# Youngju-Na/UFORecon

Measured on AMD Instinct MI355X. Metric: rays/s (per-ray volume-rendering path, 64+64 hierarchical samples, DTU-shaped 3-view 512x640), higher is better.
Workload: dtype f32; 1 GPU; configs[1]: full 512x640 frame = 327680 rays, 3 source views, 64+64 samples, rays sharded by row tiles over 1 GPU(s), depth/RGB tiles all-gathered; rays_per_frame=327680, chunk_rays=4096, side_streams=3

## Files before the change

uforecon_amd/csrc/view_transformer.hip:

```cpp
#include <cstdlib>
#include "bwd_tape.h"
#include "ufr_internal.h"
#include "weight_stream_f16.h"

namespace ufr {

template <class T>
__device__ __forceinline__ T* at32(T* base, unsigned elem) {
  typedef typename std::conditional<std::is_const<T>::value, const char, char>::type B;
  return reinterpret_cast<T*>(reinterpret_cast<B*>(base) + (elem * (unsigned)sizeof(T)));
}

template <int C, int N>
__device__ __forceinline__ void zero_tiles(f32x4 (&t)[C][N]) {
#pragma unroll
  for (int c = 0; c < C; ++c)
#pragma unroll
    for (int i = 0; i < N; ++i) t[c][i] = splat4(0.f);
}

template <int C, int VW, int VB, class WS>
__device__ __forceinline__ void layer_norm80(f32x4 (&t)[C][5], const WS& ws, int g, float eps, float asc, f32x4 (*XH)[5] = nullptr, float* RS = nullptr) {
#pragma unroll
  for (int c = 0; c < C; ++c) {
    float s = 0.f;
#pragma unroll
    for (int i = 0; i < 5; ++i) s += (t[c][i][0] + t[c][i][1]) + (t[c][i][2] + t[c][i][3]);
    const float mean = sum_groups(s) * (1.f / 80.f);
    float q = 0.f;
#pragma unroll
    for (int i = 0; i < 5; ++i)
#pragma unroll
      for (int r = 0; r < 4; ++r) {
        float d = t[c][i][r] - mean;
        q = fmaf(d, d, q);
      }
    const float rstd = fast_rsqrt(sum_groups(q) * (1.f / 80.f) + eps);
    if (RS) RS[c] = rstd * asc;
#pragma unroll
    for (int i = 0; i < 5; ++i) {
      const f32x4 gw = vec_frag<VW>(ws, i, g), gb = vec_frag<VB>(ws, i, g);
#pragma unroll
      for (int r = 0; r < 4; ++r) {
        const float xh = (t[c][i][r] - mean) * rstd;
        if (XH) XH[c][i][r] = xh;
        t[c][i][r] = xh * gw[r] + gb[r];
      }
    }
  }
}

constexpr int kVtBlock = 256;
constexpr int kVtC = 2;
constexpr int kVtMinW = 2;
constexpr int kVtOversub = 4;
constexpr int kVtWaves = kVtBlock / 64;
#ifdef UFR_PHASE_TIMING
__device__ unsigned long long g_vt_phase[32];
__device__ unsigned long long g_vt_wave[4096 * 2];
#define UFR_PHASE(i)                                                                   \
  {                                                                                    \
    const unsigned long long t_now = __builtin_readcyclecounter();                     \
    ph_acc[i] += t_now - t_prev;                                                       \
    t_prev = t_now;                                                                    \
  }
#else
#define UFR_PHASE(i)
#endif

template <int L, int C, bool LOWP, bool TAPE = false>
__global__ void __launch_bounds__(kVtBlock, kVtMinW) view_transformer_kernel(const float* __restrict__ packed,
                                                                             const float* __restrict__ x_tokens,
                                                                             const float* __restrict__ x_point,
                                                                             const float* __restrict__ rgbm,
                                                                             const float* __restrict__ dirs, int P,
                                                                             float* __restrict__ token0,
                                                                             float* __restrict__ radiance,
                                                                             float* __restrict__ view_out,
                                                                             int* __restrict__ status,
                                                                             float* __restrict__ tape = nullptr) {
  constexpr int NV = L - 1;
  constexpr int PPT = 16 / L;
  constexpr bool STRADDLE = (L == 6 && C == 2 && !TAPE);
  static_assert(!TAPE || kBlockCols % C == 0, "tape blocks");
  constexpr int PPW = STRADDLE ? 5 : PPT * C;
  constexpr bool kScoresHook = L == 4 && C == 2 && !TAPE;
  static_assert(!kScoresHook || ksteps(M_VT_V) * mat_desc(M_VT_V).n_out >= 6 * C, "the v GEMM has too few hook slots for the scores");
  extern __shared__ __attribute__((aligned(16))) char smem[];
  auto ws = wstream_f16_begin<kVtWaves, LOWP>(packed, smem);
  wstream_f16_prime<B_VT, kVtWaves>(ws);
  const int lane = threadIdx.x & 63, g = lane >> 4, j = lane & 15;
  constexpr bool kLocalScalars = (L == 6 && C == 2 && !TAPE);
  const auto sc = scalar_file<kLocalScalars, view_scalars_offset()>(ws);
  int ptw[C], tvv[C];
  bool okc[C];
#pragma unroll
  for (int c = 0; c < C; ++c) {
    if constexpr (STRADDLE) {
      ptw[c] = j < 12 ? 3 * c + j / 6 : 2;
      tvv[c] = j < 12 ? j % 6 : (c == 0 ? j - 12 : j - 8);
      okc[c] = c == 0 || j < 14;
    } else {
      ptw[c] = c * PPT + j / L;
      tvv[c] = j % L;
      okc[c] = j < PPT * L;
    }
  }
  int src[8];
#pragma unroll
  for (int s = 0; s < 8; ++s) src[s] = okc[0] ? (lane - tvv[0] + (tvv[0] + s) % L) : lane;
  int srcx[C][5];
  if constexpr (STRADDLE) {
    constexpr int kStep[6][5] = {{4, 5, 1, 2, 3}, {4, 5, 0, 2, 3}, {4, 5, 0, 1, 3}, {4, 5, 0, 1, 2}, {5, 0, 1, 2, 3}, {4, 0, 1, 2, 3}};
#pragma unroll
    for (int c = 0; c < C; ++c)
#pragma unroll
      for (int st = 0; st < 5; ++st) {
        int u = 0;
#pragma unroll
        for (int t = 0; t < 6; ++t) u = tvv[c] == t ? kStep[t][st] : u;
        const int base = j < 12 ? (j / 6) * 6 : 12;
        const int off = j < 12 ? u : (u & 3);
        srcx[c][st] = 4 * (okc[c] ? 16 * g + base + off : lane);
      }
  }
  auto exch = [&](auto ci, auto sti, float xc, float xo) __attribute__((always_inline)) -> float {
    constexpr int c = decltype(ci)::value, st = decltype(sti)::value;
    float m = xc;
    if constexpr (c == 0 && st == 0) m = j == 12 ? xo : xc;
    if constexpr (c == 0 && st == 1) m = j == 13 ? xo : xc;
    if constexpr (c == 1 && st >= 1) m = j >= 12 ? xo : xc;
    return __builtin_bit_cast(float, __builtin_amdgcn_ds_bpermute(srcx[c][st], __builtin_bit_cast(int, m)));
  };

  const int wave_global = (blockIdx.x * blockDim.x + threadIdx.x) >> 6;
  const int n_waves = (gridDim.x * blockDim.x) >> 6;
  const int n_groups = TAPE ? ((P + PPT * kBlockCols - 1) / (PPT * kBlockCols)) * (kBlockCols / C) : (P + PPW - 1) / PPW;
  const int n_iter = (n_groups + n_waves - 1) / n_waves;

#ifdef UFR_PHASE_TIMING
  unsigned long long ph_acc[12] = {};
  unsigned long long t_prev = __builtin_readcyclecounter();
  const unsigned long long t_start = t_prev;
  const unsigned long long rt_start = __builtin_amdgcn_s_memrealtime();
#endif
  for (int it = 0; it < n_iter; ++it) {
    const int grp = it * n_waves + wave_global;
    const bool wrap = it + 1 < n_iter;
    typedef ViewTapeLayout<LOWP> TapeL;
    const int col0 = __builtin_amdgcn_readfirstlane(grp < n_groups ? grp : 0) * C;
    char* const tape_blk = reinterpret_cast<char*>(tape) + (size_t)(col0 / kBlockCols) * (TapeL::block_units * 512);
    auto tape_st = [&](int tile, int c, f32x4 v) __attribute__((always_inline)) {
      if (grp < n_groups) tile_store<TapeL>(tape_blk, tile, col0 % kBlockCols + c, lane, v);
    };
    f32x4 x[C][5];
    int pidx[C];
    bool valid[C];
    auto load_x = [&](int c, f32x4 (&dst)[5]) __attribute__((always_inline)) {
      const int pp = valid[c] ? pidx[c] : 0;
      const int tv = tvv[c];
      const unsigned vrow = ((unsigned)pp * NV + (tv > 0 ? tv - 1 : 0)) * (x_point ? kViewCols : UFR_TOKEN_DIM);
      const unsigned prow_e = x_point ? (unsigned)pp * kPointCols : vrow + 32;
      const float* pbase = x_point ? x_point : x_tokens;
      const float* row = at32(x_tokens, vrow + 4 * g);
      const float* prow = at32(pbase, prow_e + 4 * g);
      const float* last = g < 2 ? prow + 32 : row + (x_point ? 32 : 72) - 8;
#pragma unroll
      for (int t = 0; t < 5; ++t) {
        f32x4 tok = vec_frag<V_VIEW_TOKEN>(ws, t, g);
        f32x4 val = ld4(t < 2 ? row + 16 * t : t < 4 ? prow + 16 * (t - 2) : last);
        dst[t] = tv == 0 ? tok : val;
        if (!valid[c]) dst[t] = splat4(0.f);
      }
    };
#pragma unroll
    for (int c = 0; c < C; ++c) {
      pidx[c] = grp * PPW + ptw[c];
      valid[c] = okc[c] && grp < n_groups && pidx[c] < P;
      load_x(c, x[c]);
    }
    track_external(x, ws);
    if constexpr (TAPE) {
#pragma unroll
      for (int c = 0; c < C; ++c)
#pragma unroll
        for (int t = 0; t < 5; ++t) tape_st(TV_X + t, c, x[c][t]);
    }
    UFR_PHASE(0)
    f32x4 q[C][5], k[C][5];
    zero_tiles(q); zero_tiles(k);
    {
      BWords<C> cur;
      const float xs_x = sc[VS_XS_X];
      split_units<0, 0, 4 * C>(x, cur, xs_x);
      static_for<3>([&](auto si) __attribute__((always_inline)) {
        constexpr int s = decltype(si)::value;
        BStep b[C];
        bwords_to_bstep(cur, b);
        if constexpr (s < 2) {
          BWords<C> nxt;
          gemm_f16_panel<M_VT_Q, s, C, kVtWaves, false>(ws, b, q, wrap, [&](auto ti) __attribute__((always_inline)) {
            constexpr int to = decltype(ti)::value;
            split_units<s + 1, to * 4 * C / 5, (to + 1) * 4 * C / 5>(x, nxt, xs_x);
          });
          gemm_f16_panel<M_VT_K, s, C, kVtWaves>(ws, b, k, wrap);
          cur = nxt;
        } else {
          gemm_f16_panel<M_VT_Q, s, C, kVtWaves>(ws, b, q, wrap);
          gemm_f16_panel<M_VT_K, s, C, kVtWaves>(ws, b, k, wrap);
        }
      });
      probe_gemm(q, ws);
      probe_gemm(k, ws);
    }
    const float q_dsc = sc[VS_Q_DSC], q_l2e = sc[VS_Q_L2E], k_dsc = sc[VS_K_DSC], k_l2e = sc[VS_K_L2E];
    if constexpr (TAPE) {
#pragma unroll
      for (int c = 0; c < C; ++c)
#pragma unroll
        for (int t = 0; t < 5; ++t) {
          tape_st(TV_Q + t, c, f32x4{elu1_acc(q[c][t][0], q_dsc, q_l2e), elu1_acc(q[c][t][1], q_dsc, q_l2e), elu1_acc(q[c][t][2], q_dsc, q_l2e), elu1_acc(q[c][t][3], q_dsc, q_l2e)});
          tape_st(TV_K + t, c, f32x4{elu1_acc(k[c][t][0], k_dsc, k_l2e), elu1_acc(k[c][t][1], k_dsc, k_l2e), elu1_acc(k[c][t][2], k_dsc, k_l2e), elu1_acc(k[c][t][3], k_dsc, k_l2e)});
        }
    }
    UFR_PHASE(1)
    float A[C][2][L], Zs[C][2];
    if constexpr (STRADDLE) {
      static_for<2>([&](auto hi) __attribute__((always_inline)) {
        constexpr int hh = decltype(hi)::value;
        float Q[C][10], K[C][10], den[C];
#pragma unroll
        for (int c = 0; c < C; ++c) {
#pragma unroll
          for (int d = 0; d < 10; ++d) {
            const int s = 10 * hh + d;
            Q[c][d] = elu1_acc(q[c][s >> 2][s & 3], q_dsc, q_l2e);
            K[c][d] = elu1_acc(k[c][s >> 2][s & 3], k_dsc, k_l2e);
          }
          float a = 0.f;
#pragma unroll
          for (int d = 0; d < 10; ++d) a = fmaf(Q[c][d], K[c][d], a);
          A[c][hh][0] = a;
          den[c] = a;
        }
        static_for<5>([&](auto sti) __attribute__((always_inline)) {
          constexpr int st = decltype(sti)::value;
          float a0 = 0.f, a1 = 0.f;
#pragma unroll
          for (int d = 0; d < 10; ++d) {
            a0 = fmaf(Q[0][d], exch(std::integral_constant<int, 0>{}, sti, K[0][d], K[1][d]), a0);
            a1 = fmaf(Q[1][d], exch(std::integral_constant<int, 1>{}, sti, K[1][d], K[0][d]), a1);
          }
          A[0][hh][1 + st] = a0; den[0] += a0;
          A[1][hh][1 + st] = a1; den[1] += a1;
        });
#pragma unroll
        for (int c = 0; c < C; ++c) Zs[c][hh] = (float)L * fast_rcp(den[c] + 1e-6f);
      });
    } else if constexpr (kScoresHook) {
    } else {
#pragma unroll
    for (int c = 0; c < C; ++c) {
#pragma unroll
      for (int hh = 0; hh < 2; ++hh) {
        float Q[10], K[10];
#pragma unroll
        for (int d = 0; d < 10; ++d) {
          const int s = 10 * hh + d;
          Q[d] = elu1_acc(q[c][s >> 2][s & 3], q_dsc, q_l2e);
          K[d] = elu1_acc(k[c][s >> 2][s & 3], k_dsc, k_l2e);
        }
        float den = 0.f;
#define UFR_ATT_STEP(S)                                                  \
        if (S < L) {                                                     \
          float a = 0.f;                                                 \
          if constexpr (L == 4 && S >= 1 && S <= 3) {                    \
            a = dot10_rot4<(S >= 1 && S <= 3) ? S : 1>(Q, K);           \
          } else {                                                       \
            _Pragma("unroll") for (int d = 0; d < 10; ++d) a = fmaf(Q[d], rot<L, S>(K[d], src), a); \
          }                                                              \
          den += a;                                                      \
          A[c][hh][S < L ? S : 0] = a;                                   \
        }
        UFR_ATT_STEP(0) UFR_ATT_STEP(1) UFR_ATT_STEP(2) UFR_ATT_STEP(3)
        UFR_ATT_STEP(4) UFR_ATT_STEP(5) UFR_ATT_STEP(6) UFR_ATT_STEP(7)
#undef UFR_ATT_STEP
        Zs[c][hh] = (float)L * fast_rcp(den + 1e-6f);
      }
    }
    }
    UFR_PHASE(2)
    f32x4 v[C][5];
    zero_tiles(v);
    if constexpr (kScoresHook) {
      float Qs[10], Ks[10];
      gemm_f16<M_VT_V, C, kVtWaves>(ws, x, v, wrap, sc[VS_XS_X], [&](auto ui) __attribute__((always_inline)) {
        constexpr int slot = decltype(ui)::value, u = slot / 3, part = slot % 3;
        if constexpr (u < 2 * C) {
          constexpr int c = u / 2, hh = u % 2;
          if constexpr (part == 0) {
#pragma unroll
            for (int d = 0; d < 10; ++d) Qs[d] = elu1_acc(q[c][(10 * hh + d) >> 2][(10 * hh + d) & 3], q_dsc, q_l2e);
          } else if constexpr (part == 1) {
#pragma unroll
            for (int d = 0; d < 10; ++d) Ks[d] = elu1_acc(k[c][(10 * hh + d) >> 2][(10 * hh + d) & 3], k_dsc, k_l2e);
          } else {
            float a0 = 0.f;
#pragma unroll
            for (int d = 0; d < 10; ++d) a0 = fmaf(Qs[d], Ks[d], a0);
            const float a1 = dot10_rot4<1>(Qs, Ks), a2 = dot10_rot4<2>(Qs, Ks), a3 = dot10_rot4<3>(Qs, Ks);
            A[c][hh][0] = a0; A[c][hh][1] = a1; A[c][hh][2] = a2; A[c][hh][3] = a3;
            Zs[c][hh] = (float)L * fast_rcp((((0.f + a0) + a1) + a2) + a3 + 1e-6f);
          }
        }
      });
    } else {
      gemm_f16<M_VT_V, C, kVtWaves>(ws, x, v, wrap, sc[VS_XS_X]);
    }
    UFR_PHASE(3)
    const float v_dsc = sc[VS_V_DSC];
    const float v_mul = v_dsc / (float)L;
    if constexpr (TAPE) {
#pragma unroll
      for (int c = 0; c < C; ++c)
#pragma unroll
        for (int t = 0; t < 5; ++t) {
          f32x4 vv;
#pragma unroll
          for (int r = 0; r < 4; ++r)
            vv[r] = (L & (L - 1)) == 0 ? v[c][t][r] * v_mul : (v[c][t][r] * v_dsc) / (float)L;
          tape_st(TV_V + t, c, vv);
        }
    }
    f32x4 msg[C][5];
    if constexpr (STRADDLE) {
      static_for<2>([&](auto hi) __attribute__((always_inline)) {
        constexpr int hh = decltype(hi)::value;
        float V[C][10], acc[C][10];
#pragma unroll
        for (int c = 0; c < C; ++c)
#pragma unroll
          for (int d = 0; d < 10; ++d) {
            const int s = 10 * hh + d;
            V[c][d] = (v[c][s >> 2][s & 3] * v_dsc) / (float)L;
            acc[c][d] = A[c][hh][0] * V[c][d];
          }
        static_for<5>([&](auto sti) __attribute__((always_inline)) {
          constexpr int st = decltype(sti)::value;
#pragma unroll
          for (int d = 0; d < 10; ++d) {
            acc[0][d] = fmaf(A[0][hh][1 + st], exch(std::integral_constant<int, 0>{}, sti, V[0][d], V[1][d]), acc[0][d]);
            acc[1][d] = fmaf(A[1][hh][1 + st], exch(std::integral_constant<int, 1>{}, sti, V[1][d], V[0][d]), acc[1][d]);
          }
        });
#pragma unroll
        for (int c = 0; c < C; ++c)
#pragma unroll
          for (int d = 0; d < 10; ++d) {
            const int s = 10 * hh + d;
            msg[c][s >> 2][s & 3] = acc[c][d] * Zs[c][hh];
          }
      });
    } else {
#pragma unroll
    for (int c = 0; c < C; ++c) {
#pragma unroll
      for (int hh = 0; hh < 2; ++hh) {
        float V[10], acc[10];
#pragma unroll
        for (int d = 0; d < 10; ++d) {
          const int s = 10 * hh + d;
          V[d] = (L & (L - 1)) == 0 ? v[c][s >> 2][s & 3] * v_mul : (v[c][s >> 2][s & 3] * v_dsc) / (float)L;
          acc[d] = 0.f;
        }
#define UFR_ATT_STEP(S)                                                  \
        if (S < L) {                                                     \
          if constexpr (L == 4 && S >= 1 && S <= 3) {                    \
            axpy10_rot4<(S >= 1 && S <= 3) ? S : 1>(acc, A[c][hh][S < L ? S : 0], V); \
          } else {                                                       \
            _Pragma("unroll") for (int d = 0; d < 10; ++d) acc[d] = fmaf(A[c][hh][S < L ? S : 0], rot<L, S>(V[d], src), acc[d]); \
          }                                                              \
        }
        UFR_ATT_STEP(0) UFR_ATT_STEP(1) UFR_ATT_STEP(2) UFR_ATT_STEP(3)
        UFR_ATT_STEP(4) UFR_ATT_STEP(5) UFR_ATT_STEP(6) UFR_ATT_STEP(7)
#undef UFR_ATT_STEP
#pragma unroll
        for (int d = 0; d < 10; ++d) {
          const int s = 10 * hh + d;
          msg[c][s >> 2][s & 3] = acc[d] * Zs[c][hh];
        }
      }
    }
    }

    UFR_PHASE(4)
    if constexpr (TAPE) {
#pragma unroll
      for (int c = 0; c < C; ++c)
#pragma unroll
        for (int t = 0; t < 5; ++t) tape_st(TV_MSG + t, c, msg[c][t]);
    }
    f32x4 m[C][5];
    zero_tiles(m);
    gemm_f16<M_VT_MERGE, C, kVtWaves>(ws, msg, m, wrap, sc[VS_M_XS]);
    UFR_PHASE(5)
    float rstd1[C] = {}, rstd2[C] = {};
    if constexpr (TAPE) {
      f32x4 xh[C][5];
      layer_norm80<C, V_VT_N1W, V_VT_N1B>(m, ws, g, sc[VS_EPS1], sc[VS_M_ASC], xh, rstd1);
#pragma unroll
      for (int c = 0; c < C; ++c)
#pragma unroll
        for (int t = 0; t < 5; ++t) { tape_st(TV_XH1 + t, c, xh[c][t]); tape_st(TV_M + t, c, m[c][t]); }
    } else {
      layer_norm80<C, V_VT_N1W, V_VT_N1B>(m, ws, g, sc[VS_EPS1], 1.f);
    }

    UFR_PHASE(6)
    f32x4 cat[C][10], hid[C][10], o[C][5];
#pragma unroll
    for (int c = 0; c < C; ++c)
#pragma unroll
      for (int t = 0; t < 5; ++t) { cat[c][t] = x[c][t]; cat[c][5 + t] = m[c][t]; }
    zero_tiles(hid);
    gemm_f16<M_VT_MLP0, C, kVtWaves>(ws, cat, hid, wrap, sc[VS_XS_X]);
    UFR_PHASE(7)
#pragma unroll
    for (int c = 0; c < C; ++c)
#pragma unroll
      for (int t = 0; t < 10; ++t)
#pragma unroll
        for (int r = 0; r < 4; ++r) hid[c][t][r] = relu_acc(hid[c][t][r]);
    unsigned relu_bits[C][2] = {};
    if constexpr (TAPE) {
#pragma unroll
      for (int c = 0; c < C; ++c)
#pragma unroll
        for (int t = 0; t < 10; ++t) {
          tape_st(TV_HID + t, c, hid[c][t] * sc[VS_MLP0_DSC]);
#pragma unroll
          for (int r = 0; r < 4; ++r)
            if (hid[c][t][r] > 0.f) relu_bits[c][(4 * t + r) >> 5] |= 1u << ((4 * t + r) & 31);
        }
    }
    zero_tiles(o);
    gemm_f16<M_VT_MLP2, C, kVtWaves>(ws, hid, o, wrap, sc[VS_M_MLP2]);
    f32x4 col[C];
    float dcomp[C];
#pragma unroll
    for (int c = 0; c < C; ++c) {
      col[c] = splat4(0.f);
      dcomp[c] = 0.f;
      const int tv = tvv[c];
      if (valid[c] && tv > 0) {
        col[c] = ld4(at32(rgbm, ((unsigned)pidx[c] * NV + (tv - 1)) * 4u));
        dcomp[c] = *at32(dirs, ((unsigned)pidx[c] * NV + (tv - 1)) * 4u + g);
      }
    }

    UFR_PHASE(8)
    if constexpr (TAPE) {
      f32x4 xh[C][5];
      layer_norm80<C, V_VT_N2W, V_VT_N2B>(o, ws, g, sc[VS_EPS2], sc[VS_MLP2_ASC], xh, rstd2);
#pragma unroll
      for (int c = 0; c < C; ++c)
#pragma unroll
        for (int t = 0; t < 5; ++t) tape_st(TV_XH2 + t, c, xh[c][t]);
    } else {
      layer_norm80<C, V_VT_N2W, V_VT_N2B>(o, ws, g, sc[VS_EPS2], 1.f);
    }
#pragma unroll
    for (int c = 0; c < C; ++c)
#pragma unroll
      for (int t = 0; t < 5; ++t)
#pragma unroll
        for (int r = 0; r < 4; ++r) o[c][t][r] += x[c][t][r];
    if constexpr (TAPE) {
#pragma unroll
      for (int c = 0; c < C; ++c) {
#pragma unroll
        for (int t = 0; t < 5; ++t) tape_st(TV_Y + t, c, o[c][t]);
        tape_st(TV_Y + 5, c, f32x4{dcomp[c], 0.f, 0.f, 0.f});
      }
    }

#pragma unroll
    for (int c = 0; c < C; ++c) {
      const int tv = tvv[c];
      if (valid[c] && tv == 0) {
#pragma unroll
        for (int t = 0; t < 5; ++t) st4(at32(token0, (unsigned)pidx[c] * UFR_TOKEN_DIM + 4 * g) + 16 * t, o[c][t]);
      }
      if (valid[c] && view_out) {
#pragma unroll
        for (int t = 0; t < 5; ++t)
          st4(at32(view_out, ((unsigned)pidx[c] * L + tv) * UFR_TOKEN_DIM + 4 * g) + 16 * t, o[c][t]);
      }
    }

    UFR_PHASE(9)
    f32x4 rin[C][6], h1[C][1], h2[C][1], lg[C][1];
#pragma unroll
    for (int c = 0; c < C; ++c) {
#pragma unroll
      for (int t = 0; t < 5; ++t) rin[c][t] = o[c][t];
      rin[c][5] = f32x4{dcomp[c], 0.f, 0.f, 0.f};
      ws.bad_out |= __builtin_amdgcn_ballot_w64(dcomp[c] != dcomp[c]);
      h1[c][0] = vec_frag<V_RW_B0>(ws, 0, g) * sc[VS_RW0_ASC];
      h2[c][0] = vec_frag<V_RW_B2>(ws, 0, g) * sc[VS_RW2_ASC];
      lg[c][0] = vec_frag<V_RW_B4>(ws, 0, g) * sc[VS_RW4_ASC];
    }
    gemm_f16<M_RW0, C, kVtWaves>(ws, rin, h1, wrap, sc[VS_RW0_XS]);
#pragma unroll
    for (int c = 0; c < C; ++c)
#pragma unroll
      for (int r = 0; r < 4; ++r) h1[c][0][r] = relu_acc(h1[c][0][r]);
    gemm_f16<M_RW2, C, kVtWaves>(ws, h1, h2, wrap, sc[VS_M_RW2]);
#pragma unroll
    for (int c = 0; c < C; ++c)
#pragma unroll
      for (int r = 0; r < 4; ++r) h2[c][0][r] = relu_acc(h2[c][0][r]);
    gemm_f16<M_RW4, C, kVtWaves>(ws, h2, lg, wrap, sc[VS_M_RW4]);
    if constexpr (TAPE) {
#pragma unroll
      for (int c = 0; c < C; ++c) {
        tape_st(TV_H1, c, h1[c][0] * sc[VS_RW0_DSC]);
        tape_st(TV_H2, c, h2[c][0] * sc[VS_RW2_DSC]);
#pragma unroll
        for (int r = 0; r < 4; ++r) {
          if (h1[c][0][r] > 0.f) relu_bits[c][1] |= 1u << (8 + r);
          if (h2[c][0][r] > 0.f) relu_bits[c][1] |= 1u << (12 + r);
        }
        const float lgt = __shfl(lg[c][0][0], j) * sc[VS_RW4_DSC];
        tape_st(TV_MISC, c, f32x4{__builtin_bit_cast(float, relu_bits[c][0]), __builtin_bit_cast(float, relu_bits[c][1]),
                                  g == 0 ? rstd1[c] : g == 1 ? lgt : 0.f, g == 0 ? rstd2[c] : 0.f});
      }
    }

    UFR_PHASE(10)
    const float rw4_dsc = sc[VS_RW4_DSC];
    if constexpr (STRADDLE) {
      float logit[C], mx[C], e[C], den[C], cr[C], cg[C], cb[C];
#pragma unroll
      for (int c = 0; c < C; ++c) {
        logit[c] = lg[c][0][0] * rw4_dsc;
        if (col[c][3] == 0.f) logit[c] = -1e9f;
        if (tvv[c] == 0) logit[c] = -INFINITY;
        mx[c] = logit[c];
      }
      static_for<5>([&](auto sti) __attribute__((always_inline)) {
        mx[0] = fmaxf(mx[0], exch(std::integral_constant<int, 0>{}, sti, logit[0], logit[1]));
        mx[1] = fmaxf(mx[1], exch(std::integral_constant<int, 1>{}, sti, logit[1], logit[0]));
      });
#pragma unroll
      for (int c = 0; c < C; ++c) {
        e[c] = tvv[c] == 0 ? 0.f : expf(logit[c] - mx[c]);
        den[c] = e[c]; cr[c] = e[c] * col[c][0]; cg[c] = e[c] * col[c][1]; cb[c] = e[c] * col[c][2];
      }
      static_for<5>([&](auto sti) __attribute__((always_inline)) {
        constexpr std::integral_constant<int, 0> c0{};
        constexpr std::integral_constant<int, 1> c1{};
        den[0] += exch(c0, sti, e[0], e[1]);
        den[1] += exch(c1, sti, e[1], e[0]);
        cr[0] += exch(c0, sti, e[0] * col[0][0], e[1] * col[1][0]);
        cr[1] += exch(c1, sti, e[1] * col[1][0], e[0] * col[0][0]);
        cg[0] += exch(c0, sti, e[0] * col[0][1], e[1] * col[1][1]);
        cg[1] += exch(c1, sti, e[1] * col[1][1], e[0] * col[0][1]);
        cb[0] += exch(c0, sti, e[0] * col[0][2], e[1] * col[1][2]);
        cb[1] += exch(c1, sti, e[1] * col[1][2], e[0] * col[0][2]);
      });
#pragma unroll
      for (int c = 0; c < C; ++c)
        if (valid[c] && tvv[c] == 0 && g == 0) {
          float* dst = at32(radiance, (unsigned)pidx[c] * 3u);
          const float rden = fast_rcp(den[c]);
          dst[0] = cr[c] * rden;
          dst[1] = cg[c] * rden;
          dst[2] = cb[c] * rden;
        }
    } else {
#pragma unroll
    for (int c = 0; c < C; ++c) {
      const int tv = tvv[c];
      float logit = lg[c][0][0] * rw4_dsc;
      if (col[c][3] == 0.f) logit = -1e9f;
      if (tv == 0) logit = -INFINITY;
      float mx = logit;
#define UFR_MAX_STEP(S) if (S < L) mx = fmaxf(mx, rot<L, S>(logit, src));
      UFR_MAX_STEP(1) UFR_MAX_STEP(2) UFR_MAX_STEP(3) UFR_MAX_STEP(4) UFR_MAX_STEP(5) UFR_MAX_STEP(6) UFR_MAX_STEP(7)
#undef UFR_MAX_STEP
      const float e = tv == 0 ? 0.f : expf(logit - mx);
      float den = e, cr = e * col[c][0], cg = e * col[c][1], cb = e * col[c][2];
#define UFR_SUM_STEP(S)                                                       \
      if (S < L) {                                                            \
        den += rot<L, S>(e, src);                                             \
        cr += rot<L, S>(e * col[c][0], src);                                  \
        cg += rot<L, S>(e * col[c][1], src);                                  \
        cb += rot<L, S>(e * col[c][2], src);                                  \
      }
      UFR_SUM_STEP(1) UFR_SUM_STEP(2) UFR_SUM_STEP(3) UFR_SUM_STEP(4) UFR_SUM_STEP(5) UFR_SUM_STEP(6) UFR_SUM_STEP(7)
#undef UFR_SUM_STEP
      if (valid[c] && tv == 0 && g == 0) {
        float* dst = at32(radiance, (unsigned)pidx[c] * 3u);
        const float rden = fast_rcp(den);
        dst[0] = cr * rden;
        dst[1] = cg * rden;
        dst[2] = cb * rden;
      }
    }
    }
    wstream_f16_finish<B_VT, kVtWaves>(ws, wrap);
    UFR_PHASE(11)
  }
  wstream_report_range(ws, status);
#ifdef UFR_PHASE_TIMING
  if (wave_global == 5 && lane == 0)
    for (int i = 0; i < 12; ++i) g_vt_phase[i] += ph_acc[i];
  if (wave_global == 5 && lane == 0) {
    g_vt_phase[20] += __builtin_amdgcn_s_memrealtime() - rt_start;
    g_vt_phase[21] += __builtin_readcyclecounter() - t_start;
  }
  if (lane == 0 && wave_global < 4096) {
    unsigned xcc;
    asm volatile("s_getreg_b32 %0, hwreg(HW_REG_XCC_ID)" : "=s"(xcc));
    unsigned hwid;
    asm volatile("s_getreg_b32 %0, hwreg(HW_REG_HW_ID)" : "=s"(hwid));
    g_vt_wave[2 * wave_global] = t_start;
    g_vt_wave[2 * wave_global + 1] = (__builtin_readcyclecounter() - t_start) | ((unsigned long long)(xcc & 0xf) << 60) |
                                     ((unsigned long long)(hwid & 0xffff) << 40);
  }
#endif
}

template <int L, bool LOWP, bool TAPE = false>
static hipError_t launch_vt(const float* packed, const float* x_tokens, const float* x_point, const float* rgb, const float* dir, int P,
                            float* token0, float* radiance, float* view_out, int* status, hipStream_t s, float* tape = nullptr) {
  constexpr int C = TAPE ? 1 : kVtC;
  constexpr int PPW = (L == 6 && C == 2 && !TAPE) ? 5 : (16 / L) * C;
  const int n_groups = TAPE ? ((P + (16 / L) * kBlockCols - 1) / ((16 / L) * kBlockCols)) * (kBlockCols / C) : (P + PPW - 1) / PPW;
  int blocks = (n_groups + kVtWaves - 1) / kVtWaves;
  constexpr int resident = 256 * (kVtMinW * 4 / kVtWaves);
  const int max_blocks = resident * kVtOversub;
  if (blocks > max_blocks) {
    const int base = (n_groups + max_blocks * kVtWaves - 1) / (max_blocks * kVtWaves);
    long best_cost = -1;
    for (int n_iter = base; n_iter <= 4 * base; ++n_iter) {
      const int b = (n_groups + kVtWaves * n_iter - 1) / (kVtWaves * n_iter);
      const long cost = (long)((b + resident - 1) / resident) * n_iter;
      if (best_cost < 0 || cost < best_cost) { best_cost = cost; blocks = b; }
    }
  }
  static LdsAttrOnce lds_attr;
  if (const hipError_t attr = lds_attr.set(reinterpret_cast<const void*>(&view_transformer_kernel<L, C, LOWP, TAPE>), kF16LdsBytes); attr != hipSuccess) return attr;
  hipLaunchKernelGGL((view_transformer_kernel<L, C, LOWP, TAPE>), dim3(blocks), dim3(kVtBlock), kF16LdsBytes, s, packed, x_tokens,
                     x_point, rgb, dir, P, token0, radiance, view_out, status, tape);
  return hipGetLastError();
}

int view_tape_blocks(int P, int NV) {
  const int PPW = (16 / (NV + 1)) * kBlockCols;
  return (P + PPW - 1) / PPW;
}
hipError_t launch_view_tape(const float* packed, const float* x_tokens, const float* rgb, const float* dir, int P, int NV,
                            float* token0, float* radiance, float* tape, bool lowp, int* status, hipStream_t s) {
  if (P <= 0 || (unsigned long long)P * (NV + 1) * UFR_TOKEN_DIM >= (1ull << 30)) return hipErrorInvalidValue;
  switch (NV) {
#define UFR_VT_CASE(N)                                                                                                   \
    case N:                                                                                                              \
      return lowp ? launch_vt<N + 1, true, true>(packed, x_tokens, nullptr, rgb, dir, P, token0, radiance, nullptr, status, s, tape) \
                  : launch_vt<N + 1, false, true>(packed, x_tokens, nullptr, rgb, dir, P, token0, radiance, nullptr, status, s, tape);
    UFR_VT_CASE(2) UFR_VT_CASE(3) UFR_VT_CASE(4) UFR_VT_CASE(5) UFR_VT_CASE(6) UFR_VT_CASE(7)
#undef UFR_VT_CASE
    default: return hipErrorInvalidValue;
  }
}

hipError_t launch_view_transformer(const float* packed, const float* x_tokens, const float* x_point, const float* rgb,
                                   const float* dir, int P, int NV, float* token0, float* radiance, float* view_out, bool lowp, int* status,
                                   hipStream_t s) {
  if (P <= 0 || (unsigned long long)P * (NV + 1) * UFR_TOKEN_DIM >= (1ull << 30)) return hipErrorInvalidValue;
  switch (NV) {
#define UFR_VT_CASE(N)                                                                                       \
    case N:                                                                                                  \
      return lowp ? launch_vt<N + 1, true>(packed, x_tokens, x_point, rgb, dir, P, token0, radiance, view_out, status, s)     \
                  : launch_vt<N + 1, false>(packed, x_tokens, x_point, rgb, dir, P, token0, radiance, view_out, status, s);
    UFR_VT_CASE(2) UFR_VT_CASE(3) UFR_VT_CASE(4) UFR_VT_CASE(5) UFR_VT_CASE(6) UFR_VT_CASE(7)
#undef UFR_VT_CASE
    default: return hipErrorInvalidValue;
  }
}

}

#ifdef UFR_PHASE_TIMING
extern "C" int ufr_debug_vt_phases(unsigned long long* out, int n, int reset) {
  unsigned long long h[32] = {};
  if (hipMemcpyFromSymbol(h, HIP_SYMBOL(ufr::g_vt_phase), sizeof(h)) != hipSuccess) return -1;
  for (int i = 0; i < n && i < 32; ++i) out[i] = h[i];
  if (reset) {
    unsigned long long z[32] = {};
    if (hipMemcpyToSymbol(HIP_SYMBOL(ufr::g_vt_phase), z, sizeof(z)) != hipSuccess) return -1;
  }
  return 0;
}
extern "C" int ufr_debug_vt_waves(unsigned long long* out, int n) {
  return hipMemcpyFromSymbol(out, HIP_SYMBOL(ufr::g_vt_wave), sizeof(unsigned long long) * n) == hipSuccess ? 0 : -1;
}
#endif
```

uforecon_amd/csrc/weight_stream_f16.h:

```cpp
#pragma once
#include <type_traits>

#include "ufr_layout_f16.h"
#include "weight_stream.h"

namespace ufr {

typedef _Float16 f16x8 __attribute__((ext_vector_type(8)));
typedef _Float16 f16x2 __attribute__((ext_vector_type(2)));
typedef float f32x2 __attribute__((ext_vector_type(2)));
typedef unsigned u32x4 __attribute__((ext_vector_type(4)));
typedef int i32x4 __attribute__((ext_vector_type(4)));

constexpr int kF16RingBytes = kF16Slots * kF16ChunkFrags * 1024;
constexpr int kF16LdsBytes = kF16RingBytes + kVecBytes;

__device__ __forceinline__ void split_pair(float a, float b, float m, unsigned& h, unsigned& l) {
  if (__builtin_constant_p(a) && __builtin_constant_p(b) && a == 0.f && b == 0.f) {
    h = l = 0u;
    return;
  }
  asm("v_fma_mixlo_f16 %0, %1, %2, 0" : "=v"(h) : "v"(a), "s"(m));
  asm("v_fma_mixhi_f16 %0, %1, %2, 0" : "+v"(h) : "v"(b), "s"(m));
  asm("v_fma_mixlo_f16 %0, %1, %2, -%3 op_sel_hi:[0,0,1]" : "=v"(l) : "v"(a), "s"(m), "v"(h));
  asm("v_fma_mixhi_f16 %0, %1, %2, -%3 op_sel:[0,0,1] op_sel_hi:[0,0,1]" : "+v"(l) : "v"(b), "s"(m), "v"(h));
}

struct BStep { f16x8 p[kPlanes]; };

typedef __bf16 bf16x2 __attribute__((ext_vector_type(2)));
typedef __bf16 bf16x8 __attribute__((ext_vector_type(8)));
__device__ __forceinline__ void split_pair_bf16(float a, float b, unsigned& h, unsigned& l) {
  h = __builtin_bit_cast(unsigned, __builtin_convertvector(f32x2{a, b}, bf16x2));
  const float ah = __builtin_bit_cast(float, h << 16), bh = __builtin_bit_cast(float, h & 0xffff0000u);
  l = __builtin_bit_cast(unsigned, __builtin_convertvector(f32x2{a - ah, b - bh}, bf16x2));
}

template <bool LOWP, bool BF16 = false, bool VORDER = false>
struct WStreamF16T {
  static constexpr bool lowp = LOWP;
  static constexpr bool bf16 = BF16;
  static constexpr bool vorder = VORDER;
  const char* src;
  char* ring;
  unsigned ring_lds;
  i32x4 rsrc;
  unsigned lds_wave;
  const f32x4* vecs;
  int wave, lane;
  unsigned long long bad_in, bad_out;
  f16x8 pre[kF16Depth][kPlanes];
};

typedef WStreamF16T<false> WStreamF16;
template <int NWAVES, bool LOWP = false, bool BF16 = false, bool VORDER = false>
__device__ __forceinline__ WStreamF16T<LOWP, BF16, VORDER> wstream_f16_begin(const float* __restrict__ packed, char* smem) {
  WStreamF16T<LOWP, BF16, VORDER> ws;
  ws.lane = threadIdx.x & 63;
  ws.wave = __builtin_amdgcn_readfirstlane(threadIdx.x >> 6);
  ws.bad_in = ws.bad_out = 0ull;
  constexpr size_t kPlaneRegion = (size_t)blob_floats() * 4;
  ws.src = reinterpret_cast<const char*>(packed) + kPlaneRegion;
  ws.ring = smem;
  ws.ring_lds = __builtin_amdgcn_readfirstlane((unsigned)(size_t)(lds_ptr_t)smem);
  {
    const unsigned long long base = reinterpret_cast<unsigned long long>(ws.src) + (unsigned long long)ws.wave * 1024ull;
    ws.rsrc[0] = __builtin_amdgcn_readfirstlane((int)(unsigned)(base & 0xffffffffull));
    ws.rsrc[1] = __builtin_amdgcn_readfirstlane((int)(unsigned)((base >> 32) & 0xffffull));
    ws.rsrc[2] = -1;
    ws.rsrc[3] = 0x00020000;
    ws.lds_wave = ws.ring_lds + (unsigned)ws.wave * 1024u;
  }
  f32x4* v = reinterpret_cast<f32x4*>(smem + kF16RingBytes);
  ws.vecs = v;
  constexpr int voff = vec_region_offset(), n4 = vec_region_floats() / 4;
  const f32x4* vs = reinterpret_cast<const f32x4*>(packed + voff);
  for (int i = threadIdx.x; i < n4; i += NWAVES * 64) v[i] = vs[i];
  __syncthreads();
  return ws;
}

template <unsigned GOFF, unsigned LOFF>
__device__ __forceinline__ void lds_dma_piece(const i32x4& rsrc, unsigned lds_wave, unsigned lane_off) {
  unsigned soff;
  asm volatile("s_add_u32 m0, %3, %5\n\ts_mov_b32 %0, %4\n\tbuffer_load_dwordx4 %1, %2, %0 offen lds"
               : "=&s"(soff)
               : "v"(lane_off), "s"(rsrc), "s"(lds_wave), "n"(GOFF), "n"(LOFF)
               : "memory", "scc");
}

template <int S, int NWAVES>
__host__ __device__ constexpr bool f16_piece_issued(int chk, int k) {
  return !f16_stream_skips_padding(S) || chk * kF16ChunkFrags + k * NWAVES < f16_stream_frags(S);
}
template <int S, int NWAVES>
__host__ __device__ constexpr int f16_chunk_pieces(int chk) {
  int n = 0;
  for (int k = 0; k < kF16ChunkFrags / NWAVES; ++k) n += f16_piece_issued<S, NWAVES>(chk, k) ? 1 : 0;
  return n;
}

template <int S, int NWAVES, int CHK, int P0 = 0, int P1 = kF16ChunkFrags / NWAVES, class WS>
__device__ __forceinline__ void wstream_f16_fetch(const WS& ws) {
  static_assert(kF16ChunkFrags % NWAVES == 0, "chunk must split evenly over the fetching waves");
  static_assert(!f16_stream_skips_padding(S) || f16_stream_frags(S) % NWAVES == 0, "a piece must be all weights or all padding");
  if constexpr (P1 > P0) {
    constexpr size_t gbase = (size_t)f16_stream_base_frags(S) * 1024;
    constexpr int soff = (CHK % kF16Slots) * (kF16ChunkFrags * 1024);
    const unsigned lane_off = ws.lane * 16;
    static_assert(gbase + (size_t)f16_stream_chunks(S) * kF16ChunkFrags * 1024 < (1ull << 31), "buffer offsets are 32-bit");
    static_for<P1 - P0>([&](auto ki) __attribute__((always_inline)) {
      constexpr unsigned k = P0 + decltype(ki)::value;
      if constexpr (f16_piece_issued<S, NWAVES>(CHK, k)) {
        constexpr int v0 = CHK * kF16ChunkFrags + k * NWAVES;
        constexpr int b0 = f16_fetch_frag(S, v0, WS::vorder);
        static_assert(f16_fetch_frag(S, v0 + NWAVES - 1, WS::vorder) == b0 + NWAVES - 1, "a piece group must be contiguous in the blob");
        lds_dma_piece<(unsigned)(gbase + (size_t)b0 * 1024), (unsigned)soff + k * NWAVES * 1024u>(ws.rsrc, ws.lds_wave, lane_off);
      }
    });
  }
}

template <int S, int NWAVES, int CHK, class WS>
__device__ __forceinline__ void wstream_f16_barrier(const WS& ws, bool wrap) {
  constexpr int n_chunks = f16_stream_chunks(S);
  constexpr int younger_pass = [] {
    int n = 0;
    for (int i = 1; i <= kF16Slots - 2; ++i)
      if (CHK + i < n_chunks) n += f16_chunk_pieces<S, NWAVES>(CHK + i);
    return n;
  }();
  constexpr int younger_wrap = [] {
    int n = 0;
    for (int i = 1; i <= kF16Slots - 2; ++i)
      if (CHK + i >= n_chunks) n += f16_chunk_pieces<S, NWAVES>((CHK + i) % n_chunks);
    return n;
  }();
  if constexpr (younger_wrap == 0) {
    asm volatile("s_waitcnt vmcnt(%0) lgkmcnt(0)" ::"n"(younger_pass) : "memory");
  } else {
    if (wrap) asm volatile("s_waitcnt vmcnt(%0) lgkmcnt(0)" ::"n"(younger_pass + younger_wrap) : "memory");
    else asm volatile("s_waitcnt vmcnt(%0) lgkmcnt(0)" ::"n"(younger_pass) : "memory");
  }
  __syncthreads();
}

template <int S, int NWAVES, int CHK, int P0 = 0, int P1 = kF16ChunkFrags / NWAVES, class WS>
__device__ __forceinline__ void wstream_f16_refill(const WS& ws, bool wrap) {
  constexpr int ahead = kF16Slots - 1, n_chunks = f16_stream_chunks(S);
  if constexpr (CHK + ahead < n_chunks) {
    wstream_f16_fetch<S, NWAVES, CHK + ahead, P0, P1>(ws);
  } else {
    if (wrap) wstream_f16_fetch<S, NWAVES, (CHK + ahead) % n_chunks, P0, P1>(ws);
  }
}

template <int S, int NWAVES, int CHK, class WS>
__device__ __forceinline__ void wstream_f16_open(const WS& ws, bool wrap) {
  wstream_f16_barrier<S, NWAVES, CHK>(ws, wrap);
  wstream_f16_refill<S, NWAVES, CHK>(ws, wrap);
}

template <int S, int NWAVES, class WS>
__device__ __forceinline__ void wstream_f16_finish(const WS& ws, bool wrap) {
  constexpr int real = f16_stream_real_chunks(S), pad = f16_stream_chunks(S) - real;
  static_for<pad>([&](auto ci) __attribute__((always_inline)) { wstream_f16_open<S, NWAVES, real + decltype(ci)::value>(ws, wrap); });
}

template <int S, int NWAVES, class WS>
__device__ __forceinline__ void wstream_f16_prime(const WS& ws) {
  static_for<kF16Slots - 1>([&](auto ci) __attribute__((always_inline)) { wstream_f16_fetch<S, NWAVES, decltype(ci)::value>(ws); });
}

template <int C, int N, class WS>
__device__ __forceinline__ void probe_gemm(const f32x4 (&out)[C][N], WS& ws) {
  bool bad = false;
#pragma unroll
  for (int c = 0; c < C; ++c) bad |= __builtin_amdgcn_class(out[c][0][0], 0x207);
  ws.bad_in |= __builtin_amdgcn_ballot_w64(bad);
}
template <int C, int N, class WS>
__device__ __forceinline__ void track_external(const f32x4 (&t)[C][N], WS& ws) {
  bool nan = false;
#pragma unroll
  for (int c = 0; c < C; ++c)
#pragma unroll
    for (int i = 0; i < N; ++i)
      nan |= __builtin_isunordered(t[c][i][0], t[c][i][1]) | __builtin_isunordered(t[c][i][2], t[c][i][3]);
  ws.bad_out |= __builtin_amdgcn_ballot_w64(nan);
}

template <class WS>
__device__ __forceinline__ void wstream_report_range(const WS& ws, int* __restrict__ status) {
  const int bits = (ws.bad_in ? 1 : 0) | (ws.bad_out ? 2 : 0);
  if (bits && ws.lane == 0) atomicOr(status, bits);
}

template <int V, class WS>
__device__ __forceinline__ f32x4 vec_frag(const WS& ws, int t, int g) {
  constexpr int base = (vec_offset(V) - vec_region_offset()) / 4;
  return ws.vecs[base + t * 4 + g];
}

__device__ __forceinline__ float uniform_f32(float v) {
  return __builtin_bit_cast(float, __builtin_amdgcn_readfirstlane(__builtin_bit_cast(int, v)));
}
template <bool LOCAL>
struct ScalarFile {
  float sv;
  __device__ __forceinline__ float operator[](int k) const {
    float v = sv;
    if constexpr (LOCAL) asm volatile("" : "+v"(v));
    return __builtin_bit_cast(float, __builtin_amdgcn_readlane(__builtin_bit_cast(int, v), k));
  }
};
template <bool LOCAL, int OFFSET, class WS>
__device__ __forceinline__ ScalarFile<LOCAL> scalar_file(const WS& ws) {
  constexpr int base = OFFSET - vec_region_offset();
  return ScalarFile<LOCAL>{reinterpret_cast<const float*>(ws.vecs)[base + (ws.lane & (kKernelScalars - 1))]};
}

__device__ __forceinline__ f32x4 mfma_f16(const f16x8& a, const f16x8& b, const f32x4& c) {
  return __builtin_amdgcn_mfma_f32_16x16x32_f16(a, b, c, 0, 0, 0);
}
template <bool BF>
__device__ __forceinline__ f32x4 mfma_planes(const f16x8& a, const f16x8& b, const f32x4& c) {
  if constexpr (BF)
    return __builtin_amdgcn_mfma_f32_16x16x32_bf16(__builtin_bit_cast(bf16x8, a), __builtin_bit_cast(bf16x8, b), c, 0, 0, 0);
  else
    return __builtin_amdgcn_mfma_f32_16x16x32_f16(a, b, c, 0, 0, 0);
}

constexpr int kHookValu = 6;
constexpr int kProducts = 3;
constexpr int kSetprio = 1;
struct NoHook {
  template <class T> __device__ __forceinline__ void operator()(T) const {}
};
template <int M, int S, int C, int NWAVES, bool SWAP = false, int STREAM = -1, int T0 = 0, int NT = mat_desc(M).n_out, class Hook = NoHook, class WS = WStreamF16>
__device__ __forceinline__ void gemm_f16_panel(WS& ws, const BStep (&b)[C], f32x4 (&out)[C][NT],
                                              bool wrap, Hook&& hook = NoHook{}) {
  constexpr bool LOWP = WS::lowp;
  constexpr bool BF = f16_mat_is_bf16(M);
  constexpr int n_planes = LOWP ? 1 : kPlanes, n_products = LOWP ? 1 : kProducts;
  constexpr int ST = STREAM >= 0 ? STREAM : f16_mat_stream(M);
  static_assert(f16_panel_index(M, S, ST) >= 0, "not a panel of the stream");
  static_assert(T0 >= 0 && NT >= 1 && T0 + NT <= mat_desc(M).n_out, "out tile range");
  constexpr int PI = f16_panel_index(M, S, ST);
  const f16x8* lds = reinterpret_cast<const f16x8*>(ws.ring) + ws.lane;
  __builtin_amdgcn_s_setprio(kSetprio);
  static_for<NT>([&](auto ti) __attribute__((always_inline)) {
    constexpr int to = decltype(ti)::value;
    constexpr int f = f16_stage_frag(ST, PI, T0 + to, WS::vorder);
    constexpr int sidx = f / kPlanes, n_stages = f16_stream_frags(ST) / kPlanes;
    __builtin_amdgcn_sched_barrier(0);
    auto read_stage = [&](auto si) __attribute__((always_inline)) {
      constexpr int s2 = decltype(si)::value, f2 = s2 * kPlanes;
      constexpr int chk = f2 / kF16ChunkFrags, in_chk = f2 % kF16ChunkFrags;
      constexpr int base = ((chk % kF16Slots) * kF16ChunkFrags + in_chk) * 64;
      constexpr int in_frags = f16_stream_frags(ST) - chk * kF16ChunkFrags;
      constexpr int n_st = (in_frags < kF16ChunkFrags ? in_frags : kF16ChunkFrags) / kPlanes, j = in_chk / kPlanes;
      constexpr int pieces = kF16ChunkFrags / NWAVES;
      if constexpr (in_chk == 0) wstream_f16_barrier<ST, NWAVES, chk>(ws, wrap);
      wstream_f16_refill<ST, NWAVES, chk, j * pieces / n_st, (j + 1) * pieces / n_st>(ws, wrap);
#pragma unroll
      for (int p = 0; p < n_planes; ++p) ws.pre[s2 % kF16Depth][p] = lds[base + p * 64];
    };
    if constexpr (sidx == 0)
      static_for<kF16Depth>([&](auto di) __attribute__((always_inline)) { read_stage(di); });
    f16x8 a[kPlanes];
#pragma unroll
    for (int p = 0; p < n_planes; ++p) a[p] = ws.pre[sidx % kF16Depth][p];
    if constexpr (sidx + kF16Depth < n_stages) read_stage(std::integral_constant<int, sidx + kF16Depth>{});
    __builtin_amdgcn_sched_barrier(0);
    hook(ti);
#pragma unroll
    for (int c = 0; c < C; ++c)
      static_for<n_products>([&](auto pi) __attribute__((always_inline)) {
        constexpr int pw[kProducts] = {1, 0, 0}, px[kProducts] = {0, 1, 0};
        constexpr int w = LOWP ? 0 : pw[decltype(pi)::value], x = LOWP ? 0 : px[decltype(pi)::value];
        out[c][to] = SWAP ? mfma_planes<BF>(b[c].p[x], a[w], out[c][to]) : mfma_planes<BF>(a[w], b[c].p[x], out[c][to]);
      });
    if constexpr (!std::is_same<std::decay_t<Hook>, NoHook>::value) {
#pragma unroll
      for (int i = 0; i < n_products * C; ++i) {
        __builtin_amdgcn_sched_group_barrier(0x008, 1, 0);
        __builtin_amdgcn_sched_group_barrier(0x002, kHookValu, 0);
      }
    }
#pragma unroll
    for (int c = 0; c < C; ++c) asm volatile("" : "+v"(out[c][to]));
  });
  __builtin_amdgcn_sched_barrier(0);
  __builtin_amdgcn_s_setprio(0);
}

template <int C>
struct BWords { unsigned w[C][kPlanes][4]; };

template <int S, int U0, int U1, bool BF = false, int C, int NIN>
__device__ __forceinline__ void split_units(const f32x4 (&in)[C][NIN], BWords<C>& bw, float m) {
  static_for<U1 - U0>([&](auto ui) __attribute__((always_inline)) {
    constexpr int u = U0 + decltype(ui)::value;
    constexpr int c = u / 4, half = (u >> 1) & 1, q = u & 1, tile = 2 * S + half;
    if constexpr (tile < NIN) {
      if constexpr (BF) split_pair_bf16(in[c][tile][2 * q], in[c][tile][2 * q + 1], bw.w[c][0][2 * half + q], bw.w[c][1][2 * half + q]);
      else split_pair(in[c][tile][2 * q], in[c][tile][2 * q + 1], m, bw.w[c][0][2 * half + q], bw.w[c][1][2 * half + q]);
    } else {
      bw.w[c][0][2 * half + q] = bw.w[c][1][2 * half + q] = 0u;
    }
  });
}

template <int C>
__device__ __forceinline__ void bwords_to_bstep(const BWords<C>& bw, BStep (&b)[C]) {
#pragma unroll
  for (int c = 0; c < C; ++c)
#pragma unroll
    for (int p = 0; p < kPlanes; ++p)
      b[c].p[p] = __builtin_bit_cast(f16x8, u32x4{bw.w[c][p][0], bw.w[c][p][1], bw.w[c][p][2], bw.w[c][p][3]});
}

__device__ __forceinline__ float elu1_acc(float a, float dsc, float dsc_l2e) {
  return a > 0.f ? __builtin_fmaf(a, dsc, 1.f) : __builtin_amdgcn_exp2f(dsc_l2e * a);
}
constexpr float kLog2e = 0x1.715476p+0f;

template <int M, int C, int NWAVES, int STREAM = -1, int NIN, class WS, class UHook = NoHook>
__device__ __forceinline__ void gemm_f16(WS& ws, const f32x4 (&in)[C][NIN], f32x4 (&out)[C][mat_desc(M).n_out],
                                        bool wrap, float m = 1.f, UHook&& uhook = NoHook{}) {
  static_assert(NIN == mat_desc(M).n_in, "input tile count");
  constexpr int n_out = mat_desc(M).n_out, NU = 4 * C;
  constexpr bool BF = f16_mat_is_bf16(M);
  constexpr bool kUser = !std::is_same<std::decay_t<UHook>, NoHook>::value;
  BWords<C> cur;
  split_units<0, 0, NU, BF>(in, cur, m);
  static_for<ksteps(M)>([&](auto si) __attribute__((always_inline)) {
    constexpr int s = decltype(si)::value;
    BStep b[C];
    bwords_to_bstep(cur, b);
    if constexpr (s + 1 < ksteps(M) && n_out >= 2) {
      BWords<C> nxt;
      gemm_f16_panel<M, s, C, NWAVES, false, STREAM>(ws, b, out, wrap, [&](auto ti) __attribute__((always_inline)) {
        constexpr int to = decltype(ti)::value;
        split_units<s + 1, to * NU / n_out, (to + 1) * NU / n_out, BF>(in, nxt, m);
        if constexpr (kUser) uhook(std::integral_constant<int, s * n_out + to>{});
      });
      cur = nxt;
    } else if constexpr (kUser) {
      gemm_f16_panel<M, s, C, NWAVES, false, STREAM>(ws, b, out, wrap, [&](auto ti) __attribute__((always_inline)) {
        uhook(std::integral_constant<int, s * n_out + decltype(ti)::value>{});
      });
      if constexpr (s + 1 < ksteps(M)) split_units<s + 1, 0, NU, BF>(in, cur, m);
    } else {
      gemm_f16_panel<M, s, C, NWAVES, false, STREAM>(ws, b, out, wrap);
      if constexpr (s + 1 < ksteps(M)) split_units<s + 1, 0, NU, BF>(in, cur, m);
    }
  });
  if constexpr (!BF) probe_gemm(out, ws);
}

}
```

Measured before the change: 2.712 million rays/s.

## Rematerialize straddle lane slots and use 16-wide MFMA for padded tail k-steps

Two independent changes. The view transformer now recomputes per-lane slot indices and bpermute sources from the lane id at each use instead of keeping them live in registers across the whole loop, which lowers register pressure. In the f16 weight-stream GEMM, the last k-step of a matrix with odd input width is half padding, so it now loads only half the fragment from LDS and issues a 16x16x16 MFMA instead of 16x16x32. The first adds recomputation ALU work, and the second relies on static layout asserts that the upper k-slots are padding.

```diff
diff --git a/uforecon_amd/csrc/view_transformer.hip b/uforecon_amd/csrc/view_transformer.hip
--- a/uforecon_amd/csrc/view_transformer.hip
+++ b/uforecon_amd/csrc/view_transformer.hip
@@ -106,24 +106,41 @@
       okc[c] = j < PPT * L;
     }
   }
+  auto slots_from_lane = [&]() __attribute__((always_inline)) {
+    int ln = lane;
+    asm volatile("" : "+v"(ln));
+    const int jj = ln & 15;
+#pragma unroll
+    for (int c = 0; c < C; ++c) {
+      ptw[c] = jj < 12 ? 3 * c + jj / 6 : 2;
+      tvv[c] = jj < 12 ? jj % 6 : (c == 0 ? jj - 12 : jj - 8);
+      okc[c] = c == 0 || jj < 14;
+    }
+  };
   int src[8];
 #pragma unroll
   for (int s = 0; s < 8; ++s) src[s] = okc[0] ? (lane - tvv[0] + (tvv[0] + s) % L) : lane;
   int srcx[C][5];
-  if constexpr (STRADDLE) {
+  auto straddle_sources = [&]() __attribute__((always_inline)) {
     constexpr int kStep[6][5] = {{4, 5, 1, 2, 3}, {4, 5, 0, 2, 3}, {4, 5, 0, 1, 3}, {4, 5, 0, 1, 2}, {5, 0, 1, 2, 3}, {4, 0, 1, 2, 3}};
-#pragma unroll
-    for (int c = 0; c < C; ++c)
+    int ln = lane;
+    asm volatile("" : "+v"(ln));
+    const int jj = ln & 15, gg = ln >> 4;
+#pragma unroll
+    for (int c = 0; c < C; ++c) {
+      const int tv = jj < 12 ? jj % 6 : (c == 0 ? jj - 12 : jj - 8);
+      const bool ok = c == 0 || jj < 14;
 #pragma unroll
       for (int st = 0; st < 5; ++st) {
         int u = 0;
 #pragma unroll
-        for (int t = 0; t < 6; ++t) u = tvv[c] == t ? kStep[t][st] : u;
-        const int base = j < 12 ? (j / 6) * 6 : 12;
-        const int off = j < 12 ? u : (u & 3);
-        srcx[c][st] = 4 * (okc[c] ? 16 * g + base + off : lane);
-      }
-  }
+        for (int t = 0; t < 6; ++t) u = tv == t ? kStep[t][st] : u;
+        const int base = jj < 12 ? (jj / 6) * 6 : 12;
+        const int off = jj < 12 ? u : (u & 3);
+        srcx[c][st] = 4 * (ok ? 16 * gg + base + off : ln);
+      }
+    }
+  };
   auto exch = [&](auto ci, auto sti, float xc, float xo) __attribute__((always_inline)) -> float {
     constexpr int c = decltype(ci)::value, st = decltype(sti)::value;
     float m = xc;
@@ -173,6 +190,7 @@
         if (!valid[c]) dst[t] = splat4(0.f);
       }
     };
+    if constexpr (STRADDLE) slots_from_lane();
 #pragma unroll
     for (int c = 0; c < C; ++c) {
       pidx[c] = grp * PPW + ptw[c];
@@ -226,6 +244,7 @@
     UFR_PHASE(1)
     float A[C][2][L], Zs[C][2];
     if constexpr (STRADDLE) {
+      straddle_sources();
       static_for<2>([&](auto hi) __attribute__((always_inline)) {
         constexpr int hh = decltype(hi)::value;
         float Q[C][10], K[C][10], den[C];
@@ -447,6 +466,14 @@
     gemm_f16<M_VT_MLP2, C, kVtWaves>(ws, hid, o, wrap, sc[VS_M_MLP2]);
     f32x4 col[C];
     float dcomp[C];
+    if constexpr (STRADDLE) {
+      slots_from_lane();
+#pragma unroll
+      for (int c = 0; c < C; ++c) {
+        pidx[c] = grp * PPW + ptw[c];
+        valid[c] = okc[c] && grp < n_groups && pidx[c] < P;
+      }
+    }
 #pragma unroll
     for (int c = 0; c < C; ++c) {
       col[c] = splat4(0.f);
@@ -540,6 +567,7 @@
     UFR_PHASE(10)
     const float rw4_dsc = sc[VS_RW4_DSC];
     if constexpr (STRADDLE) {
+      straddle_sources();
       float logit[C], mx[C], e[C], den[C], cr[C], cg[C], cb[C];
 #pragma unroll
       for (int c = 0; c < C; ++c) {
diff --git a/uforecon_amd/csrc/weight_stream_f16.h b/uforecon_amd/csrc/weight_stream_f16.h
--- a/uforecon_amd/csrc/weight_stream_f16.h
+++ b/uforecon_amd/csrc/weight_stream_f16.h
@@ -231,6 +231,42 @@
     return __builtin_amdgcn_mfma_f32_16x16x32_f16(a, b, c, 0, 0, 0);
 }
 
+__host__ __device__ constexpr bool tail16(int m, int s) { return mat_desc(m).n_in % 2 == 1 && s == ksteps(m) - 1; }
+__host__ __device__ constexpr bool tail16_upper_slots_empty(int m, int s) {
+  for (int g = 0; g < 4; ++g)
+    for (int i = 4; i < 8; ++i)
+      if (f16_col(m, s, g, i) >= 0) return false;
+  return true;
+}
+__host__ __device__ constexpr bool tail16_layout_ok() {
+  for (int m = 0; m < M_ALL_COUNT; ++m)
+    for (int s = 0; s < ksteps(m); ++s)
+      if (tail16(m, s) && !tail16_upper_slots_empty(m, s)) return false;
+  return true;
+}
+static_assert(tail16_layout_ok(), "a tail step's k-slots 4..7 must be padding in every lane group");
+__host__ __device__ constexpr bool f16_stage_tail16(int S, int stage, bool vorder) {
+  if (vorder && S == B_RT1) return false;
+  int f = stage * kPlanes;
+  for (int pi = 0; pi < f16_n_panels(S); ++pi) {
+    if (f < f16_panel_frags(S, pi)) return tail16(f16_panel(S, pi).mat, f16_panel(S, pi).s);
+    f -= f16_panel_frags(S, pi);
+  }
+  return false;
+}
+static_assert(mat_desc(M_RT_K).n_in % 2 == 0 && mat_desc(M_RT_V).n_in % 2 == 0, "B_RT1's virtual order assumes no tail step");
+
+typedef _Float16 f16x4 __attribute__((ext_vector_type(4)));
+typedef short s16x4 __attribute__((ext_vector_type(4)));
+template <bool BF>
+__device__ __forceinline__ f32x4 mfma_planes16(const f16x8& a, const f16x8& b, const f32x4& c) {
+  const f16x4 a4 = __builtin_shufflevector(a, a, 0, 1, 2, 3), b4 = __builtin_shufflevector(b, b, 0, 1, 2, 3);
+  if constexpr (BF)
+    return __builtin_amdgcn_mfma_f32_16x16x16bf16_1k(__builtin_bit_cast(s16x4, a4), __builtin_bit_cast(s16x4, b4), c, 0, 0, 0);
+  else
+    return __builtin_amdgcn_mfma_f32_16x16x16f16(a4, b4, c, 0, 0, 0);
+}
+
 constexpr int kHookValu = 6;
 constexpr int kProducts = 3;
 constexpr int kSetprio = 1;
@@ -247,12 +283,14 @@
   static_assert(f16_panel_index(M, S, ST) >= 0, "not a panel of the stream");
   static_assert(T0 >= 0 && NT >= 1 && T0 + NT <= mat_desc(M).n_out, "out tile range");
   constexpr int PI = f16_panel_index(M, S, ST);
+  constexpr bool T16 = tail16(M, S);
   const f16x8* lds = reinterpret_cast<const f16x8*>(ws.ring) + ws.lane;
   __builtin_amdgcn_s_setprio(kSetprio);
   static_for<NT>([&](auto ti) __attribute__((always_inline)) {
     constexpr int to = decltype(ti)::value;
     constexpr int f = f16_stage_frag(ST, PI, T0 + to, WS::vorder);
     constexpr int sidx = f / kPlanes, n_stages = f16_stream_frags(ST) / kPlanes;
+    static_assert(f16_stage_tail16(ST, sidx, WS::vorder) == T16, "the stage was read ahead as the panel consumes it");
     __builtin_amdgcn_sched_barrier(0);
     auto read_stage = [&](auto si) __attribute__((always_inline)) {
       constexpr int s2 = decltype(si)::value, f2 = s2 * kPlanes;
@@ -264,7 +302,14 @@
       if constexpr (in_chk == 0) wstream_f16_barrier<ST, NWAVES, chk>(ws, wrap);
       wstream_f16_refill<ST, NWAVES, chk, j * pieces / n_st, (j + 1) * pieces / n_st>(ws, wrap);
 #pragma unroll
-      for (int p = 0; p < n_planes; ++p) ws.pre[s2 % kF16Depth][p] = lds[base + p * 64];
+      for (int p = 0; p < n_planes; ++p) {
+        if constexpr (f16_stage_tail16(ST, s2, WS::vorder)) {
+          const f16x4 h = *reinterpret_cast<const f16x4*>(&lds[base + p * 64]);
+          ws.pre[s2 % kF16Depth][p] = __builtin_shufflevector(h, h, 0, 1, 2, 3, -1, -1, -1, -1);
+        } else {
+          ws.pre[s2 % kF16Depth][p] = lds[base + p * 64];
+        }
+      }
     };
     if constexpr (sidx == 0)
       static_for<kF16Depth>([&](auto di) __attribute__((always_inline)) { read_stage(di); });
@@ -279,7 +324,10 @@
       static_for<n_products>([&](auto pi) __attribute__((always_inline)) {
         constexpr int pw[kProducts] = {1, 0, 0}, px[kProducts] = {0, 1, 0};
         constexpr int w = LOWP ? 0 : pw[decltype(pi)::value], x = LOWP ? 0 : px[decltype(pi)::value];
-        out[c][to] = SWAP ? mfma_planes<BF>(b[c].p[x], a[w], out[c][to]) : mfma_planes<BF>(a[w], b[c].p[x], out[c][to]);
+        if constexpr (T16)
+          out[c][to] = SWAP ? mfma_planes16<BF>(b[c].p[x], a[w], out[c][to]) : mfma_planes16<BF>(a[w], b[c].p[x], out[c][to]);
+        else
+          out[c][to] = SWAP ? mfma_planes<BF>(b[c].p[x], a[w], out[c][to]) : mfma_planes<BF>(a[w], b[c].p[x], out[c][to]);
       });
     if constexpr (!std::is_same<std::decay_t<Hook>, NoHook>::value) {
 #pragma unroll
```

Result: no change. 2.723 million rays/s, median of 5 (+0.4%).
